# NVlabs/CenterPose

Measured on NVIDIA H100. Metric: images/sec at 512x512 DLA-34 (dla_34 + DCNv2, 7 heads, decode + PnP), higher is better.
Workload: dtype tf32x3

## Files before the change

### centerpose_b200/csrc/common.cuh

```cuda
#pragma once
#include <cuda_runtime.h>
#include <stdint.h>
#include <stdio.h>
#include <string>

#include "../../include/centerpose_b200.h"

namespace cp {

void set_error(const std::string& msg);
int fail(int code, const std::string& msg);
extern thread_local long long g_launch_counter;

#define CP_CUDA_CHECK(expr)                                                              \
  do {                                                                                   \
    cudaError_t _e = (expr);                                                             \
    if (_e != cudaSuccess)                                                               \
      return ::cp::fail(CP_ERR_CUDA, std::string(#expr) + ": " + cudaGetErrorString(_e)); \
  } while (0)

#define CP_LAUNCH_CHECK(what)                                                            \
  do {                                                                                   \
    cudaError_t _e = cudaGetLastError();                                                 \
    if (_e != cudaSuccess)                                                               \
// ... 63 lines not shown
                        int Hin, int Win, int C, int f, cudaStream_t s);
int launch_pack_conv_weight(const float* w_oihw, const float* scale, float* out, int Cout, int Cin,
                            int kh, int kw, int CoutPad, int Kpad, int ld, int colOff, cudaStream_t s,
                            int CinPad = 0);
int launch_pack_bias(const float* conv_bias, const float* bn_w, const float* bn_b, const float* bn_mean,
                     const float* bn_var, float* scale_out, float* bias_out, int C, int CPad, float eps,
                     cudaStream_t s);
int launch_pack_up_weight(const float* w_c1kk, float* out_kkc, int C, int k, cudaStream_t s);
int launch_nchw_to_nhwc(const float* in, float* out, int B, int C, int H, int W, int outStride,
                        int chanOffset, cudaStream_t s);
int launch_nhwc_to_nchw(const float* in, float* out, int B, int C, int H, int W, int inStride, cudaStream_t s);
constexpr int kGnBlocks = 64, kGnMaxGroups = 64;
inline size_t gn_workspace_doubles(int B) { return (size_t)B * kGnMaxGroups * 2 * (1 + kGnBlocks); }
int launch_group_norm_relu(float* x, const float* gamma, const float* beta, int B, int HW, int C,
                           int stride, int chanOffset, int groups, float eps, double* ws, cudaStream_t s);
int launch_gru_gates(const float* xi, const float* hh, const float* hprev, float* hout, int B_HW, int C,
                     int first_step, cudaStream_t s);

bool tma_conv_supported(const IgemmParams& p, int x3);
size_t tma_weight_bytes(int Cin, int taps, int CoutPad, int x3);
int tma_tile_n(int CoutPad, int x3);
int tma_cslab(const IgemmParams& p, int x3);
int x3_group_blocks();
int launch_pack_tma_weight(const float* src_k_by_ld, int ld, int Cin, int taps, int Cout, int CoutPad, int round_tf32,
                           int x3, int cslab, void* dst, cudaStream_t s, int bn_override = 0);
int tma_encode_nhwc_box(const float* base, int C, int W, int H, int B, int strideFloats, int boxC, int boxW, int boxH,
                        int swizzle64, void* map_out );

bool dcn_tma_supported(const IgemmParams& p, int x3);
int dcn_tma_tile_n(int CoutPad, int x3);
int dcn_tma_encode(const IgemmParams& p, int Bmax, void* map_out );
int launch_dcn_tma(const IgemmParams& p, const void* map, int x3, int round_out_tf32, cudaStream_t stream,
                   LaunchInfo* info = nullptr);
int tma_conv_encode(const IgemmParams& p, int Bmax, int x3, void* maps_out );
int launch_conv_tma(const IgemmParams& p, const void* maps, int round_out_tf32, int x3, cudaStream_t stream,
                    LaunchInfo* info = nullptr);

inline int round_up(int x, int m) { return (x + m - 1) / m * m; }

extern thread_local int g_pdl;
#ifdef __CUDACC__
__device__ __forceinline__ void griddep_wait() { asm volatile("griddepcontrol.wait;" ::: "memory"); }
__device__ __forceinline__ void griddep_launch_dependents() { asm volatile("griddepcontrol.launch_dependents;" ::: "memory"); }
template <typename... KArgs, typename... Args>
inline cudaError_t launch_kernel(void (*kern)(KArgs...), dim3 grid, dim3 block, size_t smem, cudaStream_t s, Args&&... args) {
  cudaLaunchConfig_t cfg{};
// ... 39 lines not shown
```

### centerpose_b200/csrc/conv_tma.cu

```cuda
#include <cuda.h>
#include <stdlib.h>

#include "common.cuh"
#include "umma_common.cuh"

namespace cp {
namespace {

constexpr int TM_BM = 128;
constexpr int TM_THREADS = 384;
constexpr int TM_THREADS_X3 = 512;
constexpr int TM_GROUP_X3 = 1;
}

int x3_group_blocks() {
  int g = TM_GROUP_X3;
  if (const char* e = getenv("CP_X3_GROUP")) {
    const int v = atoi(e);
    if (v >= 1 && v <= 16) g = v;
  }
  return g;
}

namespace {

struct TmaConvParams {
  CUtensorMap amap[4];
  int nsrc;
  int srcC[4];
  int B, H, W, Cin, Cout, CoutPad, BN;
  int k;
  int tile_m;
  int Wt, boxh;
  int tiles_per_image;
  long long total_tiles;
  long long m_tiles;
  uint32_t slab_bytes, slab_stride;
  int SA, SB;
  const float* bias;
  const float* residual;
  int resStride, relu, res_after_relu;
  float* out;
  int outStride, out_nchw;
  int round_tf32;
  int cslab;
  int x3;
  int group;
  const unsigned char* wtiles;
  int ksplit, sps;
  float* part;
  int fuse, tph;
  const float* fuse_w[16];
  const float* fuse_b[16];
  float* fuse_out[16];
  int fuse_cout[16];
};

using namespace umma;

struct TmaCtl {
  unsigned long long a_full[4], a_empty[4], a_split[4];
  unsigned long long b_full[8], b_empty[8];
};
static_assert(sizeof(TmaCtl) <= 512, "control block");

struct TileGeo {
  int n_tile, img, g0, r_lo;
  long long pos0;
};
__device__ __forceinline__ TileGeo decode_tile(const TmaConvParams& p, long long ct, int n_tiles) {
// ... 168 lines not shown
    if (X3) asm volatile("setmaxnreg.inc.sync.aligned.u32 208;");
    const int c = (warp - 4) >> 2, wt = tid & 127;
    float* dstage = reinterpret_cast<float*>(smem + (drain0 - smem_u32(smem))) + (size_t)c * (DRAIN_STAGE_BYTES / 4);
    const uint32_t bar_a = smem_u32(X3 ? &ctl->a_split[0] : &ctl->a_full[0]);
    const uint32_t bar_a_empty = smem_u32(&ctl->a_empty[0]);
    const uint32_t bar_b_full = smem_u32(&ctl->b_full[0]), bar_b_empty = smem_u32(&ctl->b_empty[0]);
    const uint32_t a_lo_u = p.slab_stride >> 4, b_lo_u = ((uint32_t)BN * rowb) >> 4;
    EpiParams ep;
    ep.bias = p.bias;
    ep.residual = p.residual;
    ep.resStride = p.resStride;
    ep.relu = p.relu;
    ep.res_after_relu = p.res_after_relu;
    ep.round_tf32 = p.round_tf32;
    ep.out = p.out;
    ep.outStride = p.outStride;
    ep.out_nchw = p.out_nchw;
    ep.Cout = p.Cout;
    ep.CoutPad = p.CoutPad;
    ep.H = p.H;
    ep.W = p.W;
    int sa = 0, sb = 0;
    uint32_t pa = 0, pb = 0;
    float acc[BN / 2];
    float sums[X3 ? BN / 2 : 1];
    float acc2[FUSE ? 16 : 1];
#pragma unroll
    for (int j = 0; j < BN / 2; ++j) acc[j] = 0.f;
#pragma unroll
    for (int j = 0; j < (FUSE ? 16 : 1); ++j) acc2[j] = 0.f;
    for (long long it = 0, tile = tile_at(0); tile < total_tiles; tile = tile_at(++it)) {
      const TileGeo g = decode_tile(p, tile / KS_SPLIT, n_tiles);
      const uint32_t row0 = (p.k == 3 ? (uint32_t)(g.g0 - 1 - g.r_lo * p.Wt) : 0u) + (uint32_t)c * 64u;
#pragma unroll
      for (int j = 0; j < (X3 ? BN / 2 : 1); ++j) sums[j] = 0.f;
      int kbi = 0, gk = 0;
      for (int s = 0; s < sps; ++s) {
        mbar_wait(bar_a + 8u * (uint32_t)sa, pa);
        const uint32_t a_slab = slabs0 + (uint32_t)sa * a_stage;
        for (int tap = 0; tap < taps; ++tap, ++kbi) {
          const int ky = tap / 3, kx = tap - ky * 3;
          const uint32_t arow = row0 + (p.k == 3 ? (uint32_t)(ky * p.Wt + kx) : 0u);
          mbar_wait(bar_b_full + 8u * (uint32_t)sb, pb);
          const uint64_t da = make_desc(a_slab + arow * rowb, p.cslab);
          const uint64_t db = make_desc(btiles0 + (uint32_t)sb * btile_bytes, p.cslab);
          const bool fresh = X3 ? gk == 0 : kbi == 0;
          if (p.cslab == 32)
            mma_kblock<BN, X3, false, 4>(acc, da, db, a_lo_u, b_lo_u, fresh);
          else
            mma_kblock<BN, X3, false, 2>(acc, da, db, a_lo_u, b_lo_u, fresh);
          if (wt == 0) {
            mbar_arrive(bar_b_empty + 8u * (uint32_t)sb);
            if (tap == taps - 1) mbar_arrive(bar_a_empty + 8u * (uint32_t)sa);
          }
          if (++sb == p.SB) {
            sb = 0;
            pb ^= 1u;
          }
          if (X3) {
            if (gk == p.group - 1 || kbi == KB - 1) {
#pragma unroll
              for (int j = 0; j < (X3 ? BN / 2 : 1); ++j) sums[j] += acc[X3 ? j : 0];
              gk = 0;
            } else {
              ++gk;
            }
          }
        }
        if (++sa == p.SA) {
          sa = 0;
          pa ^= 1u;
        }
      }
      const int r_me = wt >> 1;
      int n, oy, ox, m;
      const bool valid = tile_position(p, g, c * 64 + r_me, &n, &oy, &ox, &m);
      const int col_end = min(p.Cout, (g.n_tile + 1) * BN);
      const int head = FUSE ? g.n_tile / p.tph : 0, part = FUSE ? g.n_tile - head * p.tph : 0;
      if (FUSE && part == 0) {
#pragma unroll
        for (int j = 0; j < (FUSE ? 16 : 1); ++j) acc2[j] = 0.f;
      }
      auto fn = [&](int r, int cb, float (&v)[16]) {
        if (cb >= BN) return;
        if (!FUSE && KS_SPLIT > 1) {
          const long long mn = tile / KS_SPLIT;
          const int ks = (int)(tile % KS_SPLIT);
          float4* mine = reinterpret_cast<float4*>(p.part) + (((size_t)mn * KS_SPLIT + ks) * (BN >> 2) + (cb >> 2)) * p.tile_m +
                         c * 64 + r;
#pragma unroll
          for (int q = 0; q < 4; ++q) __stcg(mine + (size_t)q * p.tile_m, make_float4(v[4 * q], v[4 * q + 1], v[4 * q + 2], v[4 * q + 3]));
        } else if (FUSE) {
          const float* b1 = p.bias + (size_t)g.n_tile * BN + cb;
          const float4* w2 = reinterpret_cast<const float4*>(p.fuse_w[head]) + ((size_t)part * BN + cb) * 4;
#pragma unroll
          for (int q = 0; q < 16; ++q) {
// ... 286 lines not shown
  CP_LAUNCH_CHECK("conv_tma_kernel");
  return CP_OK;
}

int launch_conv_tma(const IgemmParams& p, const void* maps, int round_out_tf32, int x3, cudaStream_t stream,
                    LaunchInfo* info) {
  if (!p.wgt_umma) return fail(CP_ERR_INVALID, "conv_tma: weight tiles missing");
  TmaConvParams q;
  memset(&q, 0, sizeof(q));
  memcpy(q.amap, maps, sizeof(CUtensorMap) * 4);
  q.nsrc = p.nsrc;
  for (int s = 0; s < 4; ++s) q.srcC[s] = p.srcC[s];
  q.B = p.B;
  q.H = p.Hin;
  q.W = p.Win;
  q.Cin = p.Cin;
  q.Cout = p.Cout;
  q.CoutPad = p.CoutPad;
  q.BN = tma_tile_n(p.CoutPad, x3);
  if (q.BN == 0) return fail(CP_ERR_INVALID, "conv_tma: unsupported output width");
  q.x3 = x3;
  q.cslab = tma_cslab(p, x3);
  q.group = x3_group_blocks() * (32 / q.cslab);
  q.k = p.kh;
  q.Wt = p.Win + 2;
  q.tile_m = tma_tile_m(x3);
  q.boxh = tma_boxh(q.Wt, x3);
  size_t m_tiles;
  if (q.k == 3) {
    q.tiles_per_image = (p.Hin * q.Wt + q.tile_m - 1) / q.tile_m;
    m_tiles = (size_t)q.tiles_per_image * p.B;
    q.slab_bytes = (uint32_t)q.boxh * q.Wt * (uint32_t)q.cslab * 4u;
  } else {
    q.tiles_per_image = 0;
    m_tiles = ((size_t)p.B * p.Hin * p.Win + q.tile_m - 1) / q.tile_m;
    q.slab_bytes = (uint32_t)q.tile_m * (uint32_t)q.cslab * 4u;
  }
  q.slab_stride = (q.slab_bytes + 1023u) & ~1023u;
  const uint32_t btile = (uint32_t)q.BN * (uint32_t)q.cslab * 4u * (x3 ? 2u : 1u);
  const uint32_t a_stage = q.slab_stride * (x3 ? 2u : 1u);
  size_t smem = 0;
  if (int rc = tma_smem_layout(a_stage, btile, q.k, &q.SA, &q.SB, &smem)) return rc;
  q.bias = p.bias;
  q.residual = p.residual;
  q.resStride = p.resStride;
  q.relu = p.relu;
// ... 63 lines not shown
```

### centerpose_b200/csrc/dcn_tma.cu

```cuda
#include <cuda.h>
#include <stdlib.h>

#include "common.cuh"
#include "umma_common.cuh"

namespace cp {
namespace {

using namespace umma;

constexpr int DT_BM = 128;
constexpr int DT_THREADS = 512;
constexpr int DT_CS = 16;
constexpr int DT_PH = 8, DT_PW = 16;
constexpr int DT_HALO = 8;
constexpr int DT_SH = DT_PH + 2 * DT_HALO, DT_SW = DT_PW + 2 * DT_HALO;
constexpr uint32_t DT_SLAB_BYTES = DT_SH * DT_SW * DT_CS * 4;
constexpr uint32_t DT_COEF_BYTES = DT_BM * 9 * 16;

struct DcnTmaParams {
  CUtensorMap amap;
  const float* src;
  int srcStride;
  const float* offmask;
  int omStride, mask_is_logit;
  int B, H, W, Cin, Cout, CoutPad, BN;
  int tiles_x, tiles_per_image;
  long long total_tiles;
  int SB;
  int group;
  int AH;
  const float* bias;
  const float* residual;
  int resStride, relu, res_after_relu;
  float* out;
  int outStride, out_nchw, round_tf32;
  const unsigned char* wtiles;
  int ksplit, sps;
  float* part;
};

struct DcnCtl {
  unsigned long long s_full[2], s_empty[2];
  unsigned long long a_full[2], a_empty[2];
  unsigned long long c_full[2], c_empty[2];
  unsigned long long b_full[8], b_empty[8];
};

constexpr int RB_DX = 14, RB_DY = 15, RB_W = 16, RB_SLAB = 20, RB_LIVE = 21;

__device__ __forceinline__ void coef_row(const DcnTmaParams& p, const float* __restrict__ om, int oy, int ox, int ys,
                                         int xs, uint32_t dst) {
  float o[27];
// ... 267 lines not shown
    int cb = 0;
    uint32_t pc = 0;
    auto make_records = [&](long long t) {
      const long long mt = (t / KS_SPLIT) / n_tiles;
      const int im = (int)(mt / p.tiles_per_image);
      const int pt = (int)(mt - (long long)im * p.tiles_per_image);
      const int y0 = (pt / p.tiles_x) * DT_PH, x0 = (pt % p.tiles_x) * DT_PW;
      const int oy = y0 + (wt >> 4), ox = x0 + (wt & 15);
      mbar_wait(smem_u32(&ctl->c_empty[cb]), pc ^ 1u);
      coef_row(p, p.offmask + ((size_t)((size_t)im * p.H + oy) * p.W + ox) * p.omStride, oy, ox, y0 - DT_HALO, x0 - DT_HALO,
               coef0 + (uint32_t)cb * DT_COEF_BYTES + (uint32_t)wt * 144u);
      __syncwarp();
      if (lane == 0) mbar_arrive(smem_u32(&ctl->c_full[cb]));
      if (++cb == 2) {
        cb = 0;
        pc ^= 1u;
      }
    };
    if (c == 0 && (long long)blockIdx.x < total_tiles) make_records(blockIdx.x);
    const uint32_t bar_a_full = smem_u32(&ctl->a_full[0]), bar_a_empty = smem_u32(&ctl->a_empty[0]);
    const uint32_t bar_b_full = smem_u32(&ctl->b_full[0]), bar_b_empty = smem_u32(&ctl->b_empty[0]);
    int sb = 0;
    uint32_t pb = 0, cnt = 0;
    float acc[BN / 2];
    float sums[X3 ? BN / 2 : 1];
#pragma unroll
    for (int j = 0; j < BN / 2; ++j) acc[j] = 0.f;
    for (long long tile = blockIdx.x; tile < total_tiles; tile += gridDim.x) {
      if (c == 0 && tile + gridDim.x < total_tiles) make_records(tile + gridDim.x);
#pragma unroll
      for (int j = 0; j < (X3 ? BN / 2 : 1); ++j) sums[j] = 0.f;
      int gk = 0;
      for (int kbi = 0; kbi < KB; ++kbi, ++cnt) {
        const uint32_t sa = cnt & (uint32_t)(p.AH - 1);
        mbar_wait(bar_a_full + 8u * sa, (cnt >> (p.AH - 1)) & 1u);
        mbar_wait(bar_b_full + 8u * (uint32_t)sb, pb);
        const uint64_t da = make_desc(atiles0 + sa * a_stage + (uint32_t)c * 64u * 64u, DT_CS);
        const uint64_t db = make_desc(btiles0 + (uint32_t)sb * btile_bytes, DT_CS);
        mma_kblock<BN, X3, false, 2>(acc, da, db, 8192u >> 4, ((uint32_t)BN * 64u) >> 4, X3 ? gk == 0 : kbi == 0);
        if (wt == 0) {
          mbar_arrive(bar_a_empty + 8u * sa);
          mbar_arrive(bar_b_empty + 8u * (uint32_t)sb);
        }
        if (++sb == p.SB) {
          sb = 0;
          pb ^= 1u;
        }
        if (X3) {
          if (gk == p.group - 1 || kbi == KB - 1) {
#pragma unroll
            for (int j = 0; j < (X3 ? BN / 2 : 1); ++j) sums[j] += acc[X3 ? j : 0];
            gk = 0;
          } else {
            ++gk;
          }
        }
      }
      const int n_tile = (int)((tile / KS_SPLIT) % n_tiles);
      const long long m_tile = (tile / KS_SPLIT) / n_tiles;
      const int n = (int)(m_tile / p.tiles_per_image);
      const int pt = (int)(m_tile - (long long)n * p.tiles_per_image);
      const int col_end = min(p.Cout, (n_tile + 1) * BN);
      auto fn = [&](int r, int cb0, float (&v)[16]) {
        if (cb0 >= BN) return;
        const int i = c * 64 + r;
        if (KS_SPLIT > 1) {
          float4* part_row = reinterpret_cast<float4*>(p.part) + ((size_t)tile * (BN >> 2) + (cb0 >> 2)) * 128 + i;
#pragma unroll
          for (int q = 0; q < 4; ++q) __stcg(part_row + (size_t)q * 128, make_float4(v[4 * q], v[4 * q + 1], v[4 * q + 2], v[4 * q + 3]));
        } else {
          const int oy = (pt / p.tiles_x) * DT_PH + (i >> 4), ox = (pt % p.tiles_x) * DT_PW + (i & 15);
          const int m = (n * p.H + oy) * p.W + ox;
          epilogue_row<16>(ep, v, true, m, n, oy, ox, n_tile * BN + cb0, col_end);
        }
      };
      if constexpr (X3)
        drain_rows<BN>(sums, dstage, wt, 1 + c, fn);
      else
        drain_rows<BN>(acc, dstage, wt, 1 + c, fn);
    }
// ... 74 lines not shown
                   LaunchInfo* info) {
  if (!p.wgt_umma) return fail(CP_ERR_INVALID, "dcn_tma: weight tiles missing");
  if (!dcn_tma_supported(p, x3)) return fail(CP_ERR_INVALID, "dcn_tma: unsupported shape");
  DcnTmaParams q;
  memset(&q, 0, sizeof(q));
  memcpy(&q.amap, map, sizeof(CUtensorMap));
  q.src = p.src[0];
  q.srcStride = p.srcStride[0];
  q.offmask = p.offmask;
  q.omStride = p.omStride;
  q.mask_is_logit = p.mask_is_logit;
  q.B = p.B;
  q.H = p.Hin;
  q.W = p.Win;
  q.Cin = p.Cin;
  q.Cout = p.Cout;
  q.CoutPad = p.CoutPad;
  q.BN = dcn_tma_tile_n(p.CoutPad, x3);
  q.tiles_x = p.Win / DT_PW;
  q.tiles_per_image = q.tiles_x * (p.Hin / DT_PH);
  q.total_tiles = (long long)q.tiles_per_image * p.B * (p.CoutPad / q.BN);
  const uint32_t a_stage = x3 ? 16384u : 8192u;
  q.group = x3_group_blocks() * 2;
  const uint32_t btile = (uint32_t)q.BN * 64u * (x3 ? 2u : 1u);
  const size_t budget = 226 * 1024;
  q.AH = 2;
  size_t fixed = 1024 + 2 * (size_t)DT_COEF_BYTES + 1024 + 2 * (size_t)DT_SLAB_BYTES + (size_t)q.AH * a_stage +
                 2 * (size_t)DRAIN_STAGE_BYTES;
  if (fixed + 3 * (size_t)btile > budget) {
    q.AH = 1;
    fixed -= a_stage;
  }
  if (fixed + 2 * (size_t)btile > budget) return fail(CP_ERR_INVALID, "dcn_tma: tile does not fit shared memory");
  q.SB = (int)((budget - fixed) / btile);
  if (q.SB > 8) q.SB = 8;
  q.bias = p.bias;
  q.residual = p.residual;
  q.resStride = p.resStride;
  q.relu = p.relu;
  q.res_after_relu = p.res_after_relu;
  q.out = p.out;
  q.outStride = p.outStride;
  q.out_nchw = p.out_nchw;
  q.round_tf32 = round_out_tf32;
  q.wtiles = (const unsigned char*)p.wgt_umma;
  const size_t smem = fixed + (size_t)q.SB * btile;
// ... 50 lines not shown
```

### centerpose_b200/csrc/igemm_umma.cu

```cuda
#include "common.cuh"
#include "umma_common.cuh"

namespace cp {
namespace {

constexpr int UM_BM = 128;
constexpr int UM_PROD_WARPS = 8;
constexpr int UM_THREADS = (UM_PROD_WARPS + 8) * 32;
constexpr uint32_t ROW_BYTES = 128;
constexpr uint32_t A_TILE_BYTES = UM_BM * ROW_BYTES;

using namespace umma;

struct UmmaSmem {
  unsigned long long full[8];
  unsigned long long empty[8];
};

template <int PREC>
struct PrecTraits;
template <>
struct PrecTraits<0> {
  static constexpr int kElems = 64, kChunkCh = 8, kTilesA = 1;
};
template <>
struct PrecTraits<1> {
  static constexpr int kElems = 32, kChunkCh = 4, kTilesA = 2;
};

template <int PREC, int MODE, int BN>
__global__ void __launch_bounds__(UM_THREADS, 1) igemm_umma_kernel(const IgemmParams p, const int STAGES, const int NACC) {
  using T = PrecTraits<PREC>;
  extern __shared__ __align__(1024) unsigned char smem[];
  UmmaSmem* ctl = reinterpret_cast<UmmaSmem*>(smem);
  if (threadIdx.x == 0) griddep_launch_dependents();
  const uint32_t tiles0 = (smem_u32(smem) + 512u + 1023u) & ~1023u;
  const uint32_t b_tile_bytes = (uint32_t)BN * ROW_BYTES * T::kTilesA;
  const uint32_t a_bytes = A_TILE_BYTES * T::kTilesA;
  const uint32_t stage_bytes = a_bytes + b_tile_bytes;

  const int tid = threadIdx.x, warp = tid >> 5;
  const int M = p.B * p.Hout * p.Wout;
  const int n_tiles = p.CoutPad / BN;
  const int n_tile = blockIdx.x % n_tiles;
  const int m0 = (blockIdx.x / n_tiles) * UM_BM;
  const int K = p.kh * p.kw * p.Cin;
  const int KB = (K + T::kElems - 1) / T::kElems;

  if (tid == 0) {
    for (int s = 0; s < STAGES; ++s) {
      mbar_init(smem_u32(&ctl->full[s]), UM_PROD_WARPS * 32 + 1);
      mbar_init(smem_u32(&ctl->empty[s]), 2);
    }
    fence_mbar_init();
// ... 146 lines not shown
          }
        }
        fence_proxy_async_smem();
        mbar_arrive(smem_u32(&ctl->full[stage]));
        if (++stage == STAGES) {
          stage = 0;
          phase ^= 1u;
        }
      }
    }

  } else {
    const int c = (warp - UM_PROD_WARPS) >> 2, wt = tid & 127;
    constexpr bool X3 = PREC == 1;
    float acc[BN / 2];
    float sums[X3 ? BN / 2 : 1];
#pragma unroll
    for (int j = 0; j < BN / 2; ++j) acc[j] = 0.f;
#pragma unroll
    for (int j = 0; j < (X3 ? BN / 2 : 1); ++j) sums[j] = 0.f;
    int stage = 0;
    uint32_t phase = 0;
    int gk = 0;
    for (int kb = 0; kb < KB; ++kb) {
      mbar_wait(smem_u32(&ctl->full[stage]), phase);
      const uint32_t a_hi = tiles0 + (uint32_t)stage * stage_bytes;
      const uint64_t da = make_desc(a_hi + (uint32_t)c * 64u * ROW_BYTES, 32), db = make_desc(a_hi + a_bytes, 32);
      mma_kblock<BN, X3, PREC == 0, 4>(acc, da, db, A_TILE_BYTES >> 4, ((uint32_t)BN * ROW_BYTES) >> 4, X3 ? gk == 0 : kb == 0);
      if (wt == 0) mbar_arrive(smem_u32(&ctl->empty[stage]));
      if (++stage == STAGES) {
        stage = 0;
        phase ^= 1u;
      }
      if (X3) {
        if (gk == NACC - 1 || kb == KB - 1) {
#pragma unroll
          for (int j = 0; j < (X3 ? BN / 2 : 1); ++j) sums[j] += acc[X3 ? j : 0];
          gk = 0;
        } else {
          ++gk;
        }
      }
    }
    EpiParams ep;
    ep.bias = p.bias;
    ep.residual = p.residual;
    ep.resStride = p.resStride;
    ep.relu = p.relu;
    ep.res_after_relu = p.res_after_relu;
    ep.round_tf32 = 0;
    ep.out = p.out;
    ep.outStride = p.outStride;
    ep.out_nchw = p.out_nchw;
    ep.Cout = p.Cout;
    ep.CoutPad = p.CoutPad;
    ep.H = p.Hout;
    ep.W = p.Wout;
    const int col_end = min(p.Cout, (n_tile + 1) * BN);
    float* dstage = reinterpret_cast<float*>(smem + (tiles0 - smem_u32(smem)) + (size_t)STAGES * stage_bytes) +
                    (size_t)c * (DRAIN_STAGE_BYTES / 4);
    auto fn = [&](int r, int cb, float (&v)[16]) {
      const int m = m0 + c * 64 + r;
      const bool valid = m < M;
      int ox = 0, oy = 0, n = 0;
      if (valid) {
        ox = m % p.Wout;
// ... 70 lines not shown
  return (size_t)(CoutPad / bn) * KB * bn * ROW_BYTES * (prec == 0 ? 1 : 2);
}

int launch_pack_umma_weight(const float* src, int ld, int Kreal, int Cout, int CoutPad, int prec, void* dst,
                            cudaStream_t s) {
  const int elems = prec == 0 ? 64 : 32;
  const int KB = (Kreal + elems - 1) / elems;
  const int bn = umma_tile_n(CoutPad, prec);
  const int nt = CoutPad / bn;
  size_t total = (size_t)nt * KB * bn * 8;
  int blocks = (int)((total + 255) / 256);
  if (blocks > 132 * 32) blocks = 132 * 32;
  if (prec == 0)
    pack_umma_weight_kernel<0><<<blocks, 256, 0, s>>>(src, ld, Kreal, Cout, bn, nt, KB, (unsigned char*)dst);
  else
    pack_umma_weight_kernel<1><<<blocks, 256, 0, s>>>(src, ld, Kreal, Cout, bn, nt, KB, (unsigned char*)dst);
  CP_LAUNCH_CHECK("pack_umma_weight_kernel");
  return CP_OK;
}

template <int PREC, int BN>
static int launch_igemm_umma_bn(const IgemmParams& p, int stages, size_t smem, int nacc, cudaStream_t stream,
                                LaunchInfo* info) {
  void (*kern)(const IgemmParams, const int, const int) =
      (p.mode == IGEMM_DCN) ? igemm_umma_kernel<PREC, IGEMM_DCN, BN> : igemm_umma_kernel<PREC, IGEMM_NHWC_VEC, BN>;
  static PerDevice<bool, 2> configured;
  const int slot = p.mode == IGEMM_DCN ? 1 : 0;
  if (!configured.here(slot)) {
    CP_CUDA_CHECK(cudaFuncSetAttribute(kern, cudaFuncAttributeMaxDynamicSharedMemorySize, 227 * 1024));
    configured.here(slot) = true;
  }
  const int M = p.B * p.Hout * p.Wout;
  dim3 grid((unsigned)((size_t)(p.CoutPad / BN) * ((M + UM_BM - 1) / UM_BM)));
  CP_CUDA_CHECK(launch_kernel(kern, grid, dim3(UM_THREADS), smem, stream, p, stages, nacc));
  CP_LAUNCH_CHECK("igemm_umma_kernel");
  if (info) {
    info->BN = BN;
    info->ksplit = 1;
    info->grid = grid.x;
  }
  return CP_OK;
}

int launch_igemm_umma(const IgemmParams& p, int prec, cudaStream_t stream, LaunchInfo* info) {
  if (!umma_supported(p, prec)) return fail(CP_ERR_INVALID, "igemm_umma: unsupported shape");
  if (!p.wgt_umma) return fail(CP_ERR_INVALID, "igemm_umma: weight tiles missing");
  const int bn = umma_tile_n(p.CoutPad, prec);
  const int tilesA = prec == 0 ? 1 : 2;
  const size_t stage_bytes = (size_t)A_TILE_BYTES * tilesA + (size_t)bn * ROW_BYTES * tilesA;
  const size_t fixed = 512 + 1024 + 2 * (size_t)DRAIN_STAGE_BYTES;
  int stages = (int)((224 * 1024 - fixed) / stage_bytes);
  if (stages > 6) stages = 6;
  if (p.mode == IGEMM_DCN && stages > 2) stages = 2;
  if (stages < 2) return fail(CP_ERR_INVALID, "igemm_umma: tile does not fit shared memory");
  const size_t smem = fixed + stages * stage_bytes;
  const int nacc = prec == 1 ? x3_group_blocks() : 1;
  if (prec == 0) {
// ... 16 lines not shown
```

### centerpose_b200/csrc/umma_common.cuh

```cuda
#pragma once
#include <cuda.h>
#include <cuda_runtime.h>
#include <stdint.h>
#include <stdio.h>

namespace cp {
namespace umma {

__device__ __forceinline__ uint32_t smem_u32(const void* p) { return (uint32_t)__cvta_generic_to_shared(p); }

__device__ __forceinline__ void mbar_init(uint32_t bar, uint32_t count) {
  asm volatile("mbarrier.init.shared::cta.b64 [%0], %1;" ::"r"(bar), "r"(count));
}
__device__ __forceinline__ void mbar_arrive(uint32_t bar) {
  asm volatile("mbarrier.arrive.shared::cta.b64 _, [%0];" ::"r"(bar) : "memory");
}
__device__ __forceinline__ void mbar_arrive_expect_tx(uint32_t bar, uint32_t bytes) {
  asm volatile("mbarrier.arrive.expect_tx.shared::cta.b64 _, [%0], %1;" ::"r"(bar), "r"(bytes) : "memory");
}
__device__ __forceinline__ bool mbar_try_wait(uint32_t bar, uint32_t parity) {
  uint32_t ok;
  asm volatile(
      "{\n\t.reg .pred p;\n\tmbarrier.try_wait.parity.shared::cta.b64 p, [%1], %2;\n\tselp.b32 %0, 1, 0, p;\n\t}"
      : "=r"(ok)
      : "r"(bar), "r"(parity)
      : "memory");
  return ok != 0;
}
__device__ __forceinline__ void mbar_wait(uint32_t bar, uint32_t parity) {
  if (mbar_try_wait(bar, parity)) return;
  const long long t0 = clock64();
  while (!mbar_try_wait(bar, parity)) {
    if (clock64() - t0 > 4000000000LL) {
#ifdef CP_MBAR_DEBUG
      printf("wgmma kernel: mbarrier watchdog (block %d thread %d bar %u parity %u)\n", blockIdx.x, threadIdx.x, bar, parity);
#endif
      __trap();
    }
  }
}
__device__ __forceinline__ void fence_proxy_async_smem() { asm volatile("fence.proxy.async.shared::cta;" ::: "memory"); }
__device__ __forceinline__ void fence_mbar_init() { asm volatile("fence.mbarrier_init.release.cluster;" ::: "memory"); }

__device__ __forceinline__ void bulk_g2s(uint32_t dst, const void* src, uint32_t bytes, uint32_t bar) {
  asm volatile("cp.async.bulk.shared::cluster.global.mbarrier::complete_tx::bytes [%0], [%1], %2, [%3];" ::"r"(dst),
               "l"(src), "r"(bytes), "r"(bar)
               : "memory");
}
__device__ __forceinline__ void wg_bar_sync(int id) { asm volatile("bar.sync %0, 128;" ::"r"(id) : "memory"); }

__device__ __forceinline__ void wg_fence() { asm volatile("wgmma.fence.sync.aligned;" ::: "memory"); }
__device__ __forceinline__ void wg_commit() { asm volatile("wgmma.commit_group.sync.aligned;" ::: "memory"); }
template <int N>
__device__ __forceinline__ void wg_wait() { asm volatile("wgmma.wait_group.sync.aligned %0;" ::"n"(N) : "memory"); }
template <int N>
__device__ __forceinline__ void wgmma_tf32(float (&d)[N / 2], uint64_t da, uint64_t db, uint32_t scale_d);
template <int N>
__device__ __forceinline__ void wgmma_bf16(float (&d)[N / 2], uint64_t da, uint64_t db, uint32_t scale_d);
template <> __device__ __forceinline__ void wgmma_tf32<16>(float (&d)[8], uint64_t da, uint64_t db, uint32_t scale_d) {
  asm volatile(
      "{\n\t.reg .pred p;\n\tsetp.ne.b32 p, %10, 0;\n\t"
      "wgmma.mma_async.sync.aligned.m64n16k8.f32.tf32.tf32 {%0,%1,%2,%3,%4,%5,%6,%7}, %8, %9, p, 1, 1;\n\t}"
// ... 44 lines not shown
}
template <> __device__ __forceinline__ void wgmma_bf16<64>(float (&d)[32], uint64_t da, uint64_t db, uint32_t scale_d) {
  asm volatile(
      "{\n\t.reg .pred p;\n\tsetp.ne.b32 p, %34, 0;\n\t"
      "wgmma.mma_async.sync.aligned.m64n64k16.f32.bf16.bf16 {%0,%1,%2,%3,%4,%5,%6,%7,%8,%9,%10,%11,%12,%13,%14,%15,%16,%17,%18,%19,%20,%21,%22,%23,%24,%25,%26,%27,%28,%29,%30,%31}, %32, %33, p, 1, 1, 0, 0;\n\t}"
      : "+f"(d[0]), "+f"(d[1]), "+f"(d[2]), "+f"(d[3]), "+f"(d[4]), "+f"(d[5]), "+f"(d[6]), "+f"(d[7]), "+f"(d[8]), "+f"(d[9]), "+f"(d[10]), "+f"(d[11]), "+f"(d[12]), "+f"(d[13]), "+f"(d[14]), "+f"(d[15]), "+f"(d[16]), "+f"(d[17]), "+f"(d[18]), "+f"(d[19]), "+f"(d[20]), "+f"(d[21]), "+f"(d[22]), "+f"(d[23]), "+f"(d[24]), "+f"(d[25]), "+f"(d[26]), "+f"(d[27]), "+f"(d[28]), "+f"(d[29]), "+f"(d[30]), "+f"(d[31])
      : "l"(da), "l"(db), "r"(scale_d));
}
template <> __device__ __forceinline__ void wgmma_bf16<128>(float (&d)[64], uint64_t da, uint64_t db, uint32_t scale_d) {
  asm volatile(
      "{\n\t.reg .pred p;\n\tsetp.ne.b32 p, %66, 0;\n\t"
      "wgmma.mma_async.sync.aligned.m64n128k16.f32.bf16.bf16 {%0,%1,%2,%3,%4,%5,%6,%7,%8,%9,%10,%11,%12,%13,%14,%15,%16,%17,%18,%19,%20,%21,%22,%23,%24,%25,%26,%27,%28,%29,%30,%31,%32,%33,%34,%35,%36,%37,%38,%39,%40,%41,%42,%43,%44,%45,%46,%47,%48,%49,%50,%51,%52,%53,%54,%55,%56,%57,%58,%59,%60,%61,%62,%63}, %64, %65, p, 1, 1, 0, 0;\n\t}"
      : "+f"(d[0]), "+f"(d[1]), "+f"(d[2]), "+f"(d[3]), "+f"(d[4]), "+f"(d[5]), "+f"(d[6]), "+f"(d[7]), "+f"(d[8]), "+f"(d[9]), "+f"(d[10]), "+f"(d[11]), "+f"(d[12]), "+f"(d[13]), "+f"(d[14]), "+f"(d[15]), "+f"(d[16]), "+f"(d[17]), "+f"(d[18]), "+f"(d[19]), "+f"(d[20]), "+f"(d[21]), "+f"(d[22]), "+f"(d[23]), "+f"(d[24]), "+f"(d[25]), "+f"(d[26]), "+f"(d[27]), "+f"(d[28]), "+f"(d[29]), "+f"(d[30]), "+f"(d[31]), "+f"(d[32]), "+f"(d[33]), "+f"(d[34]), "+f"(d[35]), "+f"(d[36]), "+f"(d[37]), "+f"(d[38]), "+f"(d[39]), "+f"(d[40]), "+f"(d[41]), "+f"(d[42]), "+f"(d[43]), "+f"(d[44]), "+f"(d[45]), "+f"(d[46]), "+f"(d[47]), "+f"(d[48]), "+f"(d[49]), "+f"(d[50]), "+f"(d[51]), "+f"(d[52]), "+f"(d[53]), "+f"(d[54]), "+f"(d[55]), "+f"(d[56]), "+f"(d[57]), "+f"(d[58]), "+f"(d[59]), "+f"(d[60]), "+f"(d[61]), "+f"(d[62]), "+f"(d[63])
      : "l"(da), "l"(db), "r"(scale_d));
}
template <> __device__ __forceinline__ void wgmma_bf16<256>(float (&d)[128], uint64_t da, uint64_t db, uint32_t scale_d) {
  asm volatile(
      "{\n\t.reg .pred p;\n\tsetp.ne.b32 p, %130, 0;\n\t"
      "wgmma.mma_async.sync.aligned.m64n256k16.f32.bf16.bf16 {%0,%1,%2,%3,%4,%5,%6,%7,%8,%9,%10,%11,%12,%13,%14,%15,%16,%17,%18,%19,%20,%21,%22,%23,%24,%25,%26,%27,%28,%29,%30,%31,%32,%33,%34,%35,%36,%37,%38,%39,%40,%41,%42,%43,%44,%45,%46,%47,%48,%49,%50,%51,%52,%53,%54,%55,%56,%57,%58,%59,%60,%61,%62,%63,%64,%65,%66,%67,%68,%69,%70,%71,%72,%73,%74,%75,%76,%77,%78,%79,%80,%81,%82,%83,%84,%85,%86,%87,%88,%89,%90,%91,%92,%93,%94,%95,%96,%97,%98,%99,%100,%101,%102,%103,%104,%105,%106,%107,%108,%109,%110,%111,%112,%113,%114,%115,%116,%117,%118,%119,%120,%121,%122,%123,%124,%125,%126,%127}, %128, %129, p, 1, 1, 0, 0;\n\t}"
      : "+f"(d[0]), "+f"(d[1]), "+f"(d[2]), "+f"(d[3]), "+f"(d[4]), "+f"(d[5]), "+f"(d[6]), "+f"(d[7]), "+f"(d[8]), "+f"(d[9]), "+f"(d[10]), "+f"(d[11]), "+f"(d[12]), "+f"(d[13]), "+f"(d[14]), "+f"(d[15]), "+f"(d[16]), "+f"(d[17]), "+f"(d[18]), "+f"(d[19]), "+f"(d[20]), "+f"(d[21]), "+f"(d[22]), "+f"(d[23]), "+f"(d[24]), "+f"(d[25]), "+f"(d[26]), "+f"(d[27]), "+f"(d[28]), "+f"(d[29]), "+f"(d[30]), "+f"(d[31]), "+f"(d[32]), "+f"(d[33]), "+f"(d[34]), "+f"(d[35]), "+f"(d[36]), "+f"(d[37]), "+f"(d[38]), "+f"(d[39]), "+f"(d[40]), "+f"(d[41]), "+f"(d[42]), "+f"(d[43]), "+f"(d[44]), "+f"(d[45]), "+f"(d[46]), "+f"(d[47]), "+f"(d[48]), "+f"(d[49]), "+f"(d[50]), "+f"(d[51]), "+f"(d[52]), "+f"(d[53]), "+f"(d[54]), "+f"(d[55]), "+f"(d[56]), "+f"(d[57]), "+f"(d[58]), "+f"(d[59]), "+f"(d[60]), "+f"(d[61]), "+f"(d[62]), "+f"(d[63]), "+f"(d[64]), "+f"(d[65]), "+f"(d[66]), "+f"(d[67]), "+f"(d[68]), "+f"(d[69]), "+f"(d[70]), "+f"(d[71]), "+f"(d[72]), "+f"(d[73]), "+f"(d[74]), "+f"(d[75]), "+f"(d[76]), "+f"(d[77]), "+f"(d[78]), "+f"(d[79]), "+f"(d[80]), "+f"(d[81]), "+f"(d[82]), "+f"(d[83]), "+f"(d[84]), "+f"(d[85]), "+f"(d[86]), "+f"(d[87]), "+f"(d[88]), "+f"(d[89]), "+f"(d[90]), "+f"(d[91]), "+f"(d[92]), "+f"(d[93]), "+f"(d[94]), "+f"(d[95]), "+f"(d[96]), "+f"(d[97]), "+f"(d[98]), "+f"(d[99]), "+f"(d[100]), "+f"(d[101]), "+f"(d[102]), "+f"(d[103]), "+f"(d[104]), "+f"(d[105]), "+f"(d[106]), "+f"(d[107]), "+f"(d[108]), "+f"(d[109]), "+f"(d[110]), "+f"(d[111]), "+f"(d[112]), "+f"(d[113]), "+f"(d[114]), "+f"(d[115]), "+f"(d[116]), "+f"(d[117]), "+f"(d[118]), "+f"(d[119]), "+f"(d[120]), "+f"(d[121]), "+f"(d[122]), "+f"(d[123]), "+f"(d[124]), "+f"(d[125]), "+f"(d[126]), "+f"(d[127])
      : "l"(da), "l"(db), "r"(scale_d));
}

template <int BN, bool X3, bool BF16, int KS>
__device__ __forceinline__ void mma_kblock(float (&acc)[BN / 2], uint64_t da, uint64_t db, uint32_t a_lo, uint32_t b_lo,
                                           bool fresh) {
  wg_fence();
#pragma unroll
  for (int ks = 0; ks < KS; ++ks) {
    const uint32_t sd = (fresh && ks == 0) ? 0u : 1u;
    if (X3) {
      wgmma_tf32<BN>(acc, da + a_lo + 2u * ks, db + 2u * ks, sd);
      wgmma_tf32<BN>(acc, da + 2u * ks, db + b_lo + 2u * ks, 1u);
    } else if (BF16) {
      wgmma_bf16<BN>(acc, da + 2u * ks, db + 2u * ks, sd);
    } else {
      wgmma_tf32<BN>(acc, da + 2u * ks, db + 2u * ks, sd);
    }
  }
  if (X3) {
#pragma unroll
    for (int ks = 0; ks < KS; ++ks) wgmma_tf32<BN>(acc, da + 2u * ks, db + 2u * ks, 1u);
  }
  wg_commit();
  wg_wait<0>();
}

__device__ __forceinline__ float tf32_round(float x) {
  return __uint_as_float((__float_as_uint(x) + 0x1000u) & 0xffffe000u);
}
__device__ __forceinline__ uint32_t pack_bf16x2(float a, float b) {
  uint32_t r;
  asm("cvt.rn.bf16x2.f32 %0, %1, %2;" : "=r"(r) : "f"(b), "f"(a));
  return r;
}
__device__ __forceinline__ void st_shared_v4(uint32_t addr, uint32_t a, uint32_t b, uint32_t c, uint32_t d) {
  asm volatile("st.shared.v4.b32 [%0], {%1, %2, %3, %4};" ::"r"(addr), "r"(a), "r"(b), "r"(c), "r"(d) : "memory");
}
__device__ __forceinline__ void st_shared_v4f(uint32_t addr, float a, float b, float c, float d) {
  asm volatile("st.shared.v4.f32 [%0], {%1, %2, %3, %4};" ::"r"(addr), "f"(a), "f"(b), "f"(c), "f"(d) : "memory");
}
__device__ __forceinline__ float4 ld_shared_v4f(uint32_t addr) {
  float4 v;
  asm volatile("ld.shared.v4.f32 {%0,%1,%2,%3}, [%4];" : "=f"(v.x), "=f"(v.y), "=f"(v.z), "=f"(v.w) : "r"(addr) : "memory");
  return v;
}

__device__ __forceinline__ void tma_load_4d(uint32_t dst, const CUtensorMap* map, int c0, int c1, int c2, int c3, uint32_t bar) {
  asm volatile(
// ... 111 lines not shown
```

Measured before the change: 652.5.

## Overlap consecutive wgmma k-blocks with deferred retirement and dual accumulators

Replaces the issue-then-wait-all wgmma pattern with a small pipeline that keeps one k-block group in flight (wait<1>) and retires the previous block's smem stage and x3 partial-sum promotion afterwards. For x3 kernels with BN<=64 it alternates two accumulator register sets across groups, so a new group can start while the previous one finishes. This is meant to hide tensor-core drain latency between k-blocks. It costs extra registers and delays buffer releases. It also rewrites the mbarrier wait watchdog in inline PTX, and an environment variable can restore serial behaviour.

```diff
diff --git a/centerpose_b200/csrc/common.cuh b/centerpose_b200/csrc/common.cuh
--- a/centerpose_b200/csrc/common.cuh
+++ b/centerpose_b200/csrc/common.cuh
@@ -109,6 +109,7 @@
 int tma_tile_n(int CoutPad, int x3);
 int tma_cslab(const IgemmParams& p, int x3);
 int x3_group_blocks();
+int serial_kblock();
 int launch_pack_tma_weight(const float* src_k_by_ld, int ld, int Cin, int taps, int Cout, int CoutPad, int round_tf32,
                            int x3, int cslab, void* dst, cudaStream_t s, int bn_override = 0);
 int tma_encode_nhwc_box(const float* base, int C, int W, int H, int B, int strideFloats, int boxC, int boxW, int boxH,
diff --git a/centerpose_b200/csrc/conv_tma.cu b/centerpose_b200/csrc/conv_tma.cu
--- a/centerpose_b200/csrc/conv_tma.cu
+++ b/centerpose_b200/csrc/conv_tma.cu
@@ -20,6 +20,11 @@
     if (v >= 1 && v <= 16) g = v;
   }
   return g;
+}
+
+int serial_kblock() {
+  const char* e = getenv("CP_SERIAL_KBLOCK");
+  return e && atoi(e) != 0;
 }
 
 namespace {
@@ -46,6 +51,7 @@
   int cslab;
   int x3;
   int group;
+  int serial_kblock;
   const unsigned char* wtiles;
   int ksplit, sps;
   float* part;
@@ -260,13 +266,35 @@
     ep.W = p.W;
     int sa = 0, sb = 0;
     uint32_t pa = 0, pb = 0;
+    constexpr bool DUAL = X3 && BN <= 64;
     float acc[BN / 2];
+    float acc1[DUAL ? BN / 2 : 1];
     float sums[X3 ? BN / 2 : 1];
     float acc2[FUSE ? 16 : 1];
 #pragma unroll
     for (int j = 0; j < BN / 2; ++j) acc[j] = 0.f;
 #pragma unroll
+    for (int j = 0; j < (DUAL ? BN / 2 : 1); ++j) acc1[j] = 0.f;
+#pragma unroll
     for (int j = 0; j < (FUSE ? 16 : 1); ++j) acc2[j] = 0.f;
+    KPipe<X3, DUAL> pipe(p.serial_kblock != 0);
+    auto ret = [&](const KBlock& b) {
+      mbar_arrive_if(bar_b_empty + 8u * (uint32_t)b.sb, wt == 0);
+      mbar_arrive_if(bar_a_empty + 8u * (uint32_t)b.sa, wt == 0 && b.release_a);
+      if constexpr (X3) {
+        if (b.promote) {
+          fence_acc(acc);
+          fence_acc(acc1);
+          if (DUAL && b.buf) {
+#pragma unroll
+            for (int j = 0; j < BN / 2; ++j) sums[j] += acc1[DUAL ? j : 0];
+          } else {
+#pragma unroll
+            for (int j = 0; j < BN / 2; ++j) sums[j] += acc[j];
+          }
+        }
+      }
+    };
     for (long long it = 0, tile = tile_at(0); tile < total_tiles; tile = tile_at(++it)) {
       const TileGeo g = decode_tile(p, tile / KS_SPLIT, n_tiles);
       const uint32_t row0 = (p.k == 3 ? (uint32_t)(g.g0 - 1 - g.r_lo * p.Wt) : 0u) + (uint32_t)c * 64u;
@@ -274,42 +302,43 @@
       for (int j = 0; j < (X3 ? BN / 2 : 1); ++j) sums[j] = 0.f;
       int kbi = 0, gk = 0;
       for (int s = 0; s < sps; ++s) {
+        if (pipe.must_retire_first(p.SA == 1, false)) pipe.retire(ret);
         mbar_wait(bar_a + 8u * (uint32_t)sa, pa);
         const uint32_t a_slab = slabs0 + (uint32_t)sa * a_stage;
         for (int tap = 0; tap < taps; ++tap, ++kbi) {
           const int ky = tap / 3, kx = tap - ky * 3;
           const uint32_t arow = row0 + (p.k == 3 ? (uint32_t)(ky * p.Wt + kx) : 0u);
+          const bool fresh = X3 ? gk == 0 : kbi == 0;
+          if (pipe.must_retire_first(false, fresh)) pipe.retire(ret);
           mbar_wait(bar_b_full + 8u * (uint32_t)sb, pb);
           const uint64_t da = make_desc(a_slab + arow * rowb, p.cslab);
           const uint64_t db = make_desc(btiles0 + (uint32_t)sb * btile_bytes, p.cslab);
-          const bool fresh = X3 ? gk == 0 : kbi == 0;
-          if (p.cslab == 32)
-            mma_kblock<BN, X3, false, 4>(acc, da, db, a_lo_u, b_lo_u, fresh);
-          else
-            mma_kblock<BN, X3, false, 2>(acc, da, db, a_lo_u, b_lo_u, fresh);
-          if (wt == 0) {
-            mbar_arrive(bar_b_empty + 8u * (uint32_t)sb);
-            if (tap == taps - 1) mbar_arrive(bar_a_empty + 8u * (uint32_t)sa);
+          auto issue = [&](float (&a)[BN / 2]) {
+            if (p.cslab == 32)
+              mma_issue<BN, X3, false, 4>(a, da, db, a_lo_u, b_lo_u, fresh);
+            else
+              mma_issue<BN, X3, false, 2>(a, da, db, a_lo_u, b_lo_u, fresh);
+          };
+          const int buf = pipe.buf(X3 && fresh);
+          if constexpr (DUAL) {
+            if (buf) issue(acc1); else issue(acc);
+          } else {
+            issue(acc);
           }
+          const bool ends_group = X3 && (gk == p.group - 1 || kbi == KB - 1);
+          pipe.issued(ret, KBlock{sa, sb, tap == taps - 1, ends_group, buf});
           if (++sb == p.SB) {
             sb = 0;
             pb ^= 1u;
           }
-          if (X3) {
-            if (gk == p.group - 1 || kbi == KB - 1) {
-#pragma unroll
-              for (int j = 0; j < (X3 ? BN / 2 : 1); ++j) sums[j] += acc[X3 ? j : 0];
-              gk = 0;
-            } else {
-              ++gk;
-            }
-          }
+          if (X3) gk = ends_group ? 0 : gk + 1;
         }
         if (++sa == p.SA) {
           sa = 0;
           pa ^= 1u;
         }
       }
+      pipe.drain(ret);
       const int r_me = wt >> 1;
       int n, oy, ox, m;
       const bool valid = tile_position(p, g, c * 64 + r_me, &n, &oy, &ox, &m);
@@ -642,6 +671,7 @@
   q.x3 = x3;
   q.cslab = tma_cslab(p, x3);
   q.group = x3_group_blocks() * (32 / q.cslab);
+  q.serial_kblock = serial_kblock();
   q.k = p.kh;
   q.Wt = p.Win + 2;
   q.tile_m = tma_tile_m(x3);
diff --git a/centerpose_b200/csrc/dcn_tma.cu b/centerpose_b200/csrc/dcn_tma.cu
--- a/centerpose_b200/csrc/dcn_tma.cu
+++ b/centerpose_b200/csrc/dcn_tma.cu
@@ -29,6 +29,7 @@
   long long total_tiles;
   int SB;
   int group;
+  int serial_kblock;
   int AH;
   const float* bias;
   const float* residual;
@@ -342,10 +343,32 @@
     const uint32_t bar_b_full = smem_u32(&ctl->b_full[0]), bar_b_empty = smem_u32(&ctl->b_empty[0]);
     int sb = 0;
     uint32_t pb = 0, cnt = 0;
+    constexpr bool DUAL = X3 && BN <= 64;
     float acc[BN / 2];
+    float acc1[DUAL ? BN / 2 : 1];
     float sums[X3 ? BN / 2 : 1];
 #pragma unroll
     for (int j = 0; j < BN / 2; ++j) acc[j] = 0.f;
+#pragma unroll
+    for (int j = 0; j < (DUAL ? BN / 2 : 1); ++j) acc1[j] = 0.f;
+    KPipe<X3, DUAL> pipe(p.serial_kblock != 0);
+    auto ret = [&](const KBlock& b) {
+      mbar_arrive_if(bar_a_empty + 8u * (uint32_t)b.sa, wt == 0);
+      mbar_arrive_if(bar_b_empty + 8u * (uint32_t)b.sb, wt == 0);
+      if constexpr (X3) {
+        if (b.promote) {
+          fence_acc(acc);
+          fence_acc(acc1);
+          if (DUAL && b.buf) {
+#pragma unroll
+            for (int j = 0; j < BN / 2; ++j) sums[j] += acc1[DUAL ? j : 0];
+          } else {
+#pragma unroll
+            for (int j = 0; j < BN / 2; ++j) sums[j] += acc[j];
+          }
+        }
+      }
+    };
     for (long long tile = blockIdx.x; tile < total_tiles; tile += gridDim.x) {
       if (c == 0 && tile + gridDim.x < total_tiles) make_records(tile + gridDim.x);
 #pragma unroll
@@ -353,29 +376,30 @@
       int gk = 0;
       for (int kbi = 0; kbi < KB; ++kbi, ++cnt) {
         const uint32_t sa = cnt & (uint32_t)(p.AH - 1);
+        const bool fresh = X3 ? gk == 0 : kbi == 0;
+        if (pipe.must_retire_first(p.AH == 1, fresh)) pipe.retire(ret);
         mbar_wait(bar_a_full + 8u * sa, (cnt >> (p.AH - 1)) & 1u);
         mbar_wait(bar_b_full + 8u * (uint32_t)sb, pb);
         const uint64_t da = make_desc(atiles0 + sa * a_stage + (uint32_t)c * 64u * 64u, DT_CS);
         const uint64_t db = make_desc(btiles0 + (uint32_t)sb * btile_bytes, DT_CS);
-        mma_kblock<BN, X3, false, 2>(acc, da, db, 8192u >> 4, ((uint32_t)BN * 64u) >> 4, X3 ? gk == 0 : kbi == 0);
-        if (wt == 0) {
-          mbar_arrive(bar_a_empty + 8u * sa);
-          mbar_arrive(bar_b_empty + 8u * (uint32_t)sb);
-        }
+        const int buf = pipe.buf(X3 && fresh);
+        if constexpr (DUAL) {
+          if (buf)
+            mma_issue<BN, X3, false, 2>(acc1, da, db, 8192u >> 4, ((uint32_t)BN * 64u) >> 4, fresh);
+          else
+            mma_issue<BN, X3, false, 2>(acc, da, db, 8192u >> 4, ((uint32_t)BN * 64u) >> 4, fresh);
+        } else {
+          mma_issue<BN, X3, false, 2>(acc, da, db, 8192u >> 4, ((uint32_t)BN * 64u) >> 4, fresh);
+        }
+        const bool ends_group = X3 && (gk == p.group - 1 || kbi == KB - 1);
+        pipe.issued(ret, KBlock{(int)sa, sb, 1, ends_group, buf});
         if (++sb == p.SB) {
           sb = 0;
           pb ^= 1u;
         }
-        if (X3) {
-          if (gk == p.group - 1 || kbi == KB - 1) {
-#pragma unroll
-            for (int j = 0; j < (X3 ? BN / 2 : 1); ++j) sums[j] += acc[X3 ? j : 0];
-            gk = 0;
-          } else {
-            ++gk;
-          }
-        }
-      }
+        if (X3) gk = ends_group ? 0 : gk + 1;
+      }
+      pipe.drain(ret);
       const int n_tile = (int)((tile / KS_SPLIT) % n_tiles);
       const long long m_tile = (tile / KS_SPLIT) / n_tiles;
       const int n = (int)(m_tile / p.tiles_per_image);
@@ -496,6 +520,7 @@
   q.total_tiles = (long long)q.tiles_per_image * p.B * (p.CoutPad / q.BN);
   const uint32_t a_stage = x3 ? 16384u : 8192u;
   q.group = x3_group_blocks() * 2;
+  q.serial_kblock = serial_kblock();
   const uint32_t btile = (uint32_t)q.BN * 64u * (x3 ? 2u : 1u);
   const size_t budget = 226 * 1024;
   q.AH = 2;
diff --git a/centerpose_b200/csrc/igemm_umma.cu b/centerpose_b200/csrc/igemm_umma.cu
--- a/centerpose_b200/csrc/igemm_umma.cu
+++ b/centerpose_b200/csrc/igemm_umma.cu
@@ -29,7 +29,8 @@
 };
 
 template <int PREC, int MODE, int BN>
-__global__ void __launch_bounds__(UM_THREADS, 1) igemm_umma_kernel(const IgemmParams p, const int STAGES, const int NACC) {
+__global__ void __launch_bounds__(UM_THREADS, 1) igemm_umma_kernel(const IgemmParams p, const int STAGES, const int NACC,
+                                                                       const int serial) {
   using T = PrecTraits<PREC>;
   extern __shared__ __align__(1024) unsigned char smem[];
   UmmaSmem* ctl = reinterpret_cast<UmmaSmem*>(smem);
@@ -222,26 +223,33 @@
     int stage = 0;
     uint32_t phase = 0;
     int gk = 0;
+    KPipe<X3, false> pipe(serial != 0);
+    auto ret = [&](const KBlock& b) {
+      mbar_arrive_if(smem_u32(&ctl->empty[b.sb]), wt == 0);
+      if constexpr (X3) {
+        if (b.promote) {
+          fence_acc(acc);
+#pragma unroll
+          for (int j = 0; j < BN / 2; ++j) sums[j] += acc[j];
+        }
+      }
+    };
     for (int kb = 0; kb < KB; ++kb) {
+      const bool fresh = X3 ? gk == 0 : kb == 0;
+      if (pipe.must_retire_first(false, fresh)) pipe.retire(ret);
       mbar_wait(smem_u32(&ctl->full[stage]), phase);
       const uint32_t a_hi = tiles0 + (uint32_t)stage * stage_bytes;
       const uint64_t da = make_desc(a_hi + (uint32_t)c * 64u * ROW_BYTES, 32), db = make_desc(a_hi + a_bytes, 32);
-      mma_kblock<BN, X3, PREC == 0, 4>(acc, da, db, A_TILE_BYTES >> 4, ((uint32_t)BN * ROW_BYTES) >> 4, X3 ? gk == 0 : kb == 0);
-      if (wt == 0) mbar_arrive(smem_u32(&ctl->empty[stage]));
+      mma_issue<BN, X3, PREC == 0, 4>(acc, da, db, A_TILE_BYTES >> 4, ((uint32_t)BN * ROW_BYTES) >> 4, fresh);
+      const bool ends_group = X3 && (gk == NACC - 1 || kb == KB - 1);
+      pipe.issued(ret, KBlock{0, stage, 0, ends_group, 0});
       if (++stage == STAGES) {
         stage = 0;
         phase ^= 1u;
       }
-      if (X3) {
-        if (gk == NACC - 1 || kb == KB - 1) {
-#pragma unroll
-          for (int j = 0; j < (X3 ? BN / 2 : 1); ++j) sums[j] += acc[X3 ? j : 0];
-          gk = 0;
-        } else {
-          ++gk;
-        }
-      }
-    }
+      if (X3) gk = ends_group ? 0 : gk + 1;
+    }
+    pipe.drain(ret);
     EpiParams ep;
     ep.bias = p.bias;
     ep.residual = p.residual;
@@ -358,7 +366,7 @@
 template <int PREC, int BN>
 static int launch_igemm_umma_bn(const IgemmParams& p, int stages, size_t smem, int nacc, cudaStream_t stream,
                                 LaunchInfo* info) {
-  void (*kern)(const IgemmParams, const int, const int) =
+  void (*kern)(const IgemmParams, const int, const int, const int) =
       (p.mode == IGEMM_DCN) ? igemm_umma_kernel<PREC, IGEMM_DCN, BN> : igemm_umma_kernel<PREC, IGEMM_NHWC_VEC, BN>;
   static PerDevice<bool, 2> configured;
   const int slot = p.mode == IGEMM_DCN ? 1 : 0;
@@ -368,7 +376,7 @@
   }
   const int M = p.B * p.Hout * p.Wout;
   dim3 grid((unsigned)((size_t)(p.CoutPad / BN) * ((M + UM_BM - 1) / UM_BM)));
-  CP_CUDA_CHECK(launch_kernel(kern, grid, dim3(UM_THREADS), smem, stream, p, stages, nacc));
+  CP_CUDA_CHECK(launch_kernel(kern, grid, dim3(UM_THREADS), smem, stream, p, stages, nacc, serial_kblock()));
   CP_LAUNCH_CHECK("igemm_umma_kernel");
   if (info) {
     info->BN = BN;
diff --git a/centerpose_b200/csrc/umma_common.cuh b/centerpose_b200/csrc/umma_common.cuh
--- a/centerpose_b200/csrc/umma_common.cuh
+++ b/centerpose_b200/csrc/umma_common.cuh
@@ -15,6 +15,11 @@
 __device__ __forceinline__ void mbar_arrive(uint32_t bar) {
   asm volatile("mbarrier.arrive.shared::cta.b64 _, [%0];" ::"r"(bar) : "memory");
 }
+__device__ __forceinline__ void mbar_arrive_if(uint32_t bar, bool pred) {
+  asm volatile("{\n\t.reg .pred p;\n\tsetp.ne.b32 p, %1, 0;\n\t@p mbarrier.arrive.shared::cta.b64 _, [%0];\n\t}" ::"r"(bar),
+               "r"((uint32_t)pred)
+               : "memory");
+}
 __device__ __forceinline__ void mbar_arrive_expect_tx(uint32_t bar, uint32_t bytes) {
   asm volatile("mbarrier.arrive.expect_tx.shared::cta.b64 _, [%0], %1;" ::"r"(bar), "r"(bytes) : "memory");
 }
@@ -28,16 +33,33 @@
   return ok != 0;
 }
 __device__ __forceinline__ void mbar_wait(uint32_t bar, uint32_t parity) {
+#ifndef CP_MBAR_DEBUG
+  asm volatile(
+      "{\n\t.reg .pred p;\n\t.reg .s64 t0, t1;\n\t"
+      "mbarrier.try_wait.parity.shared::cta.b64 p, [%0], %1;\n\t"
+      "@p bra MBW_DONE;\n\t"
+      "mov.u64 t0, %%clock64;\n"
+      "MBW_LOOP:\n\t"
+      "mbarrier.try_wait.parity.shared::cta.b64 p, [%0], %1;\n\t"
+      "@p bra MBW_DONE;\n\t"
+      "mov.u64 t1, %%clock64;\n\t"
+      "sub.s64 t1, t1, t0;\n\t"
+      "setp.gt.s64 p, t1, 4000000000;\n\t"
+      "@p trap;\n\t"
+      "bra MBW_LOOP;\n"
+      "MBW_DONE:\n\t}" ::"r"(bar),
+      "r"(parity)
+      : "memory");
+#else
   if (mbar_try_wait(bar, parity)) return;
   const long long t0 = clock64();
   while (!mbar_try_wait(bar, parity)) {
     if (clock64() - t0 > 4000000000LL) {
-#ifdef CP_MBAR_DEBUG
       printf("wgmma kernel: mbarrier watchdog (block %d thread %d bar %u parity %u)\n", blockIdx.x, threadIdx.x, bar, parity);
+      __trap();
+    }
+  }
 #endif
-      __trap();
-    }
-  }
 }
 __device__ __forceinline__ void fence_proxy_async_smem() { asm volatile("fence.proxy.async.shared::cta;" ::: "memory"); }
 __device__ __forceinline__ void fence_mbar_init() { asm volatile("fence.mbarrier_init.release.cluster;" ::: "memory"); }
@@ -128,9 +150,16 @@
       : "l"(da), "l"(db), "r"(scale_d));
 }
 
+template <int N>
+__device__ __forceinline__ void fence_acc(float (&d)[N]) {
+#pragma unroll
+  for (int j = 0; j < N; ++j) asm volatile("" : "+f"(d[j])::"memory");
+}
+
 template <int BN, bool X3, bool BF16, int KS>
-__device__ __forceinline__ void mma_kblock(float (&acc)[BN / 2], uint64_t da, uint64_t db, uint32_t a_lo, uint32_t b_lo,
-                                           bool fresh) {
+__device__ __forceinline__ void mma_issue(float (&acc)[BN / 2], uint64_t da, uint64_t db, uint32_t a_lo, uint32_t b_lo,
+                                          bool fresh) {
+  fence_acc(acc);
   wg_fence();
 #pragma unroll
   for (int ks = 0; ks < KS; ++ks) {
@@ -149,8 +178,61 @@
     for (int ks = 0; ks < KS; ++ks) wgmma_tf32<BN>(acc, da + 2u * ks, db + 2u * ks, 1u);
   }
   wg_commit();
+  fence_acc(acc);
+}
+
+template <int BN, bool X3, bool BF16, int KS>
+__device__ __forceinline__ void mma_kblock(float (&acc)[BN / 2], uint64_t da, uint64_t db, uint32_t a_lo, uint32_t b_lo,
+                                           bool fresh) {
+  mma_issue<BN, X3, BF16, KS>(acc, da, db, a_lo, b_lo, fresh);
   wg_wait<0>();
-}
+  fence_acc(acc);
+}
+
+struct KBlock {
+  int sa, sb;
+  int release_a;
+  int promote;
+  int buf;
+};
+template <bool X3, bool DUAL>
+struct KPipe {
+  bool serial;
+  bool pending = false;
+  KBlock last{};
+  int group = 0;
+  __device__ __forceinline__ explicit KPipe(bool s) : serial(s) {}
+  __device__ __forceinline__ bool must_retire_first(bool needs_prev_stage, bool fresh) const {
+    return pending && (needs_prev_stage || (X3 && !DUAL && fresh));
+  }
+  template <class Ret>
+  __device__ __forceinline__ void retire(Ret&& ret) {
+    wg_wait<0>();
+    ret(last);
+    pending = false;
+  }
+  __device__ __forceinline__ int buf(bool fresh) {
+    if (DUAL && fresh) group ^= 1;
+    return DUAL ? group : 0;
+  }
+  template <class Ret>
+  __device__ __forceinline__ void issued(Ret&& ret, const KBlock& b) {
+    if (pending) {
+      wg_wait<1>();
+      ret(last);
+    }
+    last = b;
+    pending = true;
+    if (serial) retire(ret);
+  }
+  template <class Ret>
+  __device__ __forceinline__ void drain(Ret&& ret) {
+    wg_wait<0>();
+    if (pending) ret(last);
+    pending = false;
+    group = 0;
+  }
+};
 
 __device__ __forceinline__ float tf32_round(float x) {
   return __uint_as_float((__float_as_uint(x) + 0x1000u) & 0xffffe000u);
```

New measurement: 667.3 (median of 6 runs). 1.02x the previous value.
